# Windere/EAS-SNN

Hardware: AMD Instinct MI355X
Metric: event-frames/sec (T=3) SYOLOX-S Gen1 304x240 (higher is better)
Workload: dtype f32

## Files before the change

### eas_snn_amd/csrc/conv_wgrad_mfma.hip

```cpp
#include <stdio.h>
#include <stdlib.h>

#include "eas_common.h"

namespace {

typedef __bf16 bf16x8 __attribute__((ext_vector_type(8)));
typedef short s16x4 __attribute__((ext_vector_type(4)));
typedef float f32x16 __attribute__((ext_vector_type(16)));
typedef __attribute__((address_space(3))) s16x4 lds_s16x4;

constexpr int TP = 80;
constexpr int KST = TP / 16;
#ifndef EAS_WG_COMMIT_KS
#define EAS_WG_COMMIT_KS (KST - 2)
#endif
constexpr int COMMIT_KS = EAS_WG_COMMIT_KS;
constexpr int ROWB = 64;
constexpr int A_PLANE = TP * ROWB;

__device__ __attribute__((aligned(16))) float eas_wg_zero_page[4] = {0.f, 0.f, 0.f, 0.f};

struct WgGeom {
    int NI, Cin, Cout, Hi, Wi, Ho, Wo;
    int RT, rows_seg, nseg, rows_in, RS, Q;
    int total_rows, ntiles, kslices;
    int ci_blocks;
    int pitchX, pitchY;
    int parts, Wst, lpad, qshift, hv;
    int pn;
    int single;
    int nit;
};

__device__ __forceinline__ void split3(float v, __bf16& hi, __bf16& mid, __bf16& lo) {
    hi = (__bf16)v;
    const float r1 = v - (float)hi;
    mid = (__bf16)r1;
    const float r2 = r1 - (float)mid;
    lo = (__bf16)r2;
}

__device__ __forceinline__ bf16x8 tr_frag(const unsigned char* p0, const unsigned char* p1) {
    const s16x4 a = __builtin_amdgcn_ds_read_tr16_b64_v4i16((lds_s16x4*)p0);
    const s16x4 b = __builtin_amdgcn_ds_read_tr16_b64_v4i16((lds_s16x4*)p1);
    return __builtin_bit_cast(bf16x8, __builtin_shufflevector(a, b, 0, 1, 2, 3, 4, 5, 6, 7));
}

template <int NTERMS>
__device__ __forceinline__ void stage_terms(unsigned char* dst, int term_stride, const float (&v)[8]) {
    if constexpr (NTERMS == 1) {
        bf16x8 t0;
#pragma unroll
        for (int j = 0; j < 8; ++j) t0[j] = (__bf16)v[j];
        *(bf16x8*)dst = t0;
    } else {
        bf16x8 t0, t1, t2;
#pragma unroll
        for (int j = 0; j < 8; ++j) {
            __bf16 a, b, c;
            split3(v[j], a, b, c);
            t0[j] = a;
            t1[j] = b;
            t2[j] = c;
        }
        *(bf16x8*)dst = t0;
        *(bf16x8*)(dst + term_stride) = t1;
        *(bf16x8*)(dst + 2 * term_stride) = t2;
    }
}

template <int S, int XT, int PM, int PN, int VEC, bool XPL, int NITX = 0>
__device__ __forceinline__ void conv_wgrad_body(const float* __restrict__ x, const float* __restrict__ gy, float* __restrict__ slabs,
                                                const WgGeom& g, unsigned char* smem, const int bx, const int by) {
    static_assert(!XPL || XT == 1, "spike planes are one exact bf16 term");
    typedef float vecf __attribute__((ext_vector_type(VEC)));
    typedef unsigned int u32x4 __attribute__((ext_vector_type(4)));
    constexpr int NW = 3 * PM * PN, NT = 64 * NW, NIT = NITX ? NITX : (PM * PN == 4 ? 1 : 2);
    constexpr int A_TERM = PM * A_PLANE, A_BYTES = 3 * A_TERM;
    const int tid = threadIdx.x, lane = tid & 63, wave = tid >> 6;
    const int kh = wave % 3, pair = wave / 3, pm = pair / PN, pn = pair % PN;
    const int cob = by / g.ci_blocks, cib = by - cob * g.ci_blocks;
    const int co0 = cob * 32 * PM, ci0 = cib * 32 * PN;
    const int b_plane = g.Q * ROWB, b_term = PN * b_plane;
    const int buf_bytes = A_BYTES + XT * b_term;
    const int npix = g.RT * g.Wo;

    if (g.parts == 1) {
        const int rows = g.nseg * g.rows_in;
        for (int i = tid; i < rows * 2 * 4 * PN * XT * (g.single ? 1 : 2); i += NT) {
            int rest = i;
            const int piece = rest & 3; rest >>= 2;
            const int side = rest & 1; rest >>= 1;
            const int row = rest % rows; rest /= rows;
            const int pl = rest % (PN * XT), buf = rest / (PN * XT);
            const int col = side ? g.RS - 1 : 0;
            *(uint4*)(smem + (size_t)buf * buf_bytes + A_BYTES + (size_t)pl * b_plane + ((size_t)row * g.RS + col) * ROWB + piece * 16) =
                make_uint4(0, 0, 0, 0);
        }
    }

    if (PN == 1 && g.Cin - ci0 < 32) {
        const int ng = (g.Cin - ci0 + 7) / 8;
        for (int i = tid; i < g.Q * (4 - ng) * XT * (g.single ? 1 : 2); i += NT) {
            int rest = i;
            const int grp = ng + rest % (4 - ng); rest /= (4 - ng);
            const int q = rest % g.Q; rest /= g.Q;
            const int t = rest % XT, buf = rest / XT;
            *(uint4*)(smem + (size_t)buf * buf_bytes + A_BYTES + (size_t)t * b_term + (size_t)q * ROWB + grp * 16) = make_uint4(0, 0, 0, 0);
        }
    }

    const int gq = lane >> 4, li = lane & 15, qrow = li >> 2, pcol = li & 3;
    const int lane_col_bytes = ((gq & 1) * 16 + 4 * pcol) * 2;
    const int kb = (gq >> 1) * 8 + qrow;
    const int a_lane = pm * A_PLANE + kb * ROWB + lane_col_bytes;
    int b_lane[KST][2];
#pragma unroll
    for (int ks = 0; ks < KST; ++ks)
#pragma unroll
        for (int rd = 0; rd < 2; ++rd) {
            const int p = ks * 16 + kb + 4 * rd;
            int q = 0;
            if (p < npix) {
                const int rl = p / g.Wo, c = p - rl * g.Wo;
                const int seg = rl / g.rows_seg, rr = rl - seg * g.rows_seg;
                q = (seg * g.rows_in + rr * S) * g.RS + c * S + g.qshift;
            }
            b_lane[ks][rd] = A_BYTES + pn * b_plane + q * ROWB + lane_col_bytes;
        }

    const int unitsA = TP / VEC, nA = unitsA * 4 * PM;
    const int nbg = PN == 1 ? (g.Cin - ci0 >= 32 ? 4 : (g.Cin - ci0 + 7) / 8) : 4 * PN;
    const int units_row = g.Wst / VEC, units_seg = g.rows_in * units_row, unitsB = g.nseg * units_seg, nB = unitsB * nbg;
    const int part = g.parts > 1 ? bx % g.parts : 0;
    const int ycol0 = part * g.Wo;
    const int xcol0 = g.parts > 1 ? ycol0 * S - g.hv : 0;
    const int nitems = nA + nB;
    const size_t planeY = (size_t)g.Ho * g.pitchY, planeX = (size_t)g.Hi * g.pitchX;
    constexpr bool BUF = XT == 1;
    constexpr unsigned OOB = 0x80000000u;
    int it_kind[NIT], it_seg[NIT], it_row[NIT], it_lofs[NIT];
    unsigned it_off[BUF ? NIT : 1];
    int it_col[BUF ? 1 : NIT], it_ch[BUF ? 1 : NIT];
#pragma unroll
    for (int it = 0; it < NIT; ++it) {
        int id = it * NT + tid;
        id = id < nitems ? id : nitems - 1;
        if (id < nA) {
            const int u = id / (4 * PM), gi = id - u * (4 * PM);
            const int p0 = u * VEC;
            const int rl = p0 / g.Wo, c = p0 - rl * g.Wo;
            it_kind[it] = p0 < npix ? 0 : 2;
            it_seg[it] = rl / g.rows_seg;
            it_row[it] = rl - it_seg[it] * g.rows_seg;
            const int ch = co0 + gi * 8;
            if constexpr (BUF) {
                it_off[it] = (p0 < npix && ch < g.Cout)
                                 ? (unsigned)((((size_t)it_seg[it] * g.Cout + ch) * g.Ho + it_row[it]) * g.pitchY + ycol0 + c) * 4u : OOB;
            } else {
                it_col[it] = c;
                it_ch[it] = gi * 8;
            }
            it_lofs[it] = (gi >> 2) * A_PLANE + p0 * ROWB + (gi & 3) * 16;
        } else {
            const int idb = id - nA;
            const int u = idb / nbg, gi = idb - u * nbg;
            const int seg = u / units_seg, rem = u - seg * units_seg;
            const int rl = rem / units_row, cu = rem - rl * units_row;
            it_kind[it] = 1;
            it_seg[it] = seg;
            it_row[it] = rl;
            const int ch = ci0 + gi * 8, gc = xcol0 + cu * VEC;
            if constexpr (BUF) {
                const bool sok = ch < g.Cin && gc >= 0 && gc < g.pitchX;
                it_off[it] = !sok ? OOB
                             : XPL ? (unsigned)((((size_t)seg * (g.Cin / 8) + (ch >> 3)) * g.Hi + rl) * g.pitchX + gc) * 16u
                                   : (unsigned)((((size_t)seg * g.Cin + ch) * g.Hi + rl) * g.pitchX + gc) * 4u;
            } else {
                it_col[it] = cu * VEC;
                it_ch[it] = gi * 8;
            }
            it_lofs[it] = A_BYTES + (gi >> 2) * b_plane + ((seg * g.rows_in + rl) * g.RS + g.lpad + cu * VEC) * ROWB + (gi & 3) * 16;
        }
    }

    vecf L[NIT][8];
    constexpr bool UNI = NIT == 1;
    u32x4 LP[UNI ? 1 : NIT][(XPL && !UNI) ? VEC : 1];
    const unsigned planeYb = (unsigned)planeY * 4u, planeXb = (unsigned)planeX * 4u;
    auto fetch = [&](int it, int tile) {
        const int rho0 = (g.parts > 1 ? tile / g.parts : tile) * g.RT;
        const int img0 = rho0 / g.Ho, r0 = rho0 - img0 * g.Ho;
        if constexpr (!BUF) {
            const int img = img0 + it_seg[it];
            const float* src;
            size_t plane;
            bool ok;
            if (it_kind[it] == 1) {
                const int ir = r0 * S - 1 + it_row[it];
                const int gc = xcol0 + it_col[it];
                ok = ir >= 0 && ir < g.Hi && img < g.NI && ci0 + it_ch[it] < g.Cin && gc >= 0 && gc < g.pitchX;
                const int ch = ci0 + it_ch[it] < g.Cin ? ci0 + it_ch[it] : g.Cin - 8;
                src = x + (((size_t)(ok ? img : 0) * g.Cin + ch) * g.Hi + (ok ? ir : 0)) * g.pitchX + (ok ? gc : 0);
                plane = planeX;
            } else {
                ok = it_kind[it] == 0 && img < g.NI && co0 + it_ch[it] < g.Cout;
                const int ch = co0 + it_ch[it] < g.Cout ? co0 + it_ch[it] : g.Cout - 8;
                src = gy + (((size_t)(ok ? img : 0) * g.Cout + ch) * g.Ho + (ok ? r0 + it_row[it] : 0)) * g.pitchY + (ok ? ycol0 + it_col[it] : 0);
                plane = planeY;
            }
            const float* sp = ok ? src : eas_wg_zero_page;
            const size_t cs = ok ? plane : 0;
#pragma unroll
            for (int j = 0; j < 8; ++j) L[it][j] = *(const vecf*)(sp + j * cs);
        } else {
        const bool img_ok = img0 + it_seg[it] < g.NI;
        if (it_kind[it] == 1) {
            const int r0s = r0 * S - 1;
            const bool ok = img_ok && (unsigned)(r0s + it_row[it]) < (unsigned)g.Hi;
            const unsigned voff = ok ? it_off[it] : OOB;
            if constexpr (XPL) {
                const char* base = reinterpret_cast<const char*>(x) + (((long)img0 * (g.Cin / 8)) * g.Hi + r0s) * (long)g.pitchX * 16;
                const __amdgpu_buffer_rsrc_t rs = __builtin_amdgcn_make_buffer_rsrc((void*)base, 0, OOB, 0x00020000);
#pragma unroll
                for (int p = 0; p < VEC; ++p) {
                    const u32x4 v = __builtin_amdgcn_raw_buffer_load_b128(rs, voff + 16 * p, 0, 0);
                    if constexpr (!UNI) {
                        LP[it][p] = v;
                    } else if constexpr (VEC == 4) {
                        L[it][p] = __builtin_bit_cast(vecf, v);
                    } else {
                        typedef unsigned int u32x2 __attribute__((ext_vector_type(2)));
                        L[it][2 * p] = __builtin_bit_cast(vecf, (u32x2)__builtin_shufflevector(v, v, 0, 1));
                        L[it][2 * p + 1] = __builtin_bit_cast(vecf, (u32x2)__builtin_shufflevector(v, v, 2, 3));
                    }
                }
            } else {
                const char* base = reinterpret_cast<const char*>(x) + (((long)img0 * g.Cin) * g.Hi + r0s) * (long)g.pitchX * 4;
                const __amdgpu_buffer_rsrc_t rs = __builtin_amdgcn_make_buffer_rsrc((void*)base, 0, OOB, 0x00020000);
#pragma unroll
                for (int j = 0; j < 8; ++j) {
                    if constexpr (VEC == 4) L[it][j] = __builtin_bit_cast(vecf, __builtin_amdgcn_raw_buffer_load_b128(rs, voff, j * planeXb, 0));
                    else L[it][j] = __builtin_bit_cast(vecf, __builtin_amdgcn_raw_buffer_load_b64(rs, voff, j * planeXb, 0));
                }
            }
        } else {
            const unsigned voff = img_ok ? it_off[it] : OOB;
            const char* base = reinterpret_cast<const char*>(gy) + (((long)img0 * g.Cout) * g.Ho + r0) * (long)g.pitchY * 4;
            const __amdgpu_buffer_rsrc_t rs = __builtin_amdgcn_make_buffer_rsrc((void*)base, 0, OOB, 0x00020000);
#pragma unroll
            for (int j = 0; j < 8; ++j) {
                if constexpr (VEC == 4) L[it][j] = __builtin_bit_cast(vecf, __builtin_amdgcn_raw_buffer_load_b128(rs, voff, j * planeYb, 0));
                else L[it][j] = __builtin_bit_cast(vecf, __builtin_amdgcn_raw_buffer_load_b64(rs, voff, j * planeYb, 0));
            }
        }
        }
    };
    auto commit = [&](unsigned char* buf, int it) {
        if (XPL && it_kind[it] == 1) {
#pragma unroll
            for (int p = 0; p < VEC; ++p) {
                if constexpr (!UNI) {
                    *(u32x4*)(buf + it_lofs[it] + p * ROWB) = LP[it][p];
                } else if constexpr (VEC == 4) {
                    *(vecf*)(buf + it_lofs[it] + p * ROWB) = L[it][p];
                } else {
                    *(vecf*)(buf + it_lofs[it] + p * ROWB) = L[it][2 * p];
                    *(vecf*)(buf + it_lofs[it] + p * ROWB + 8) = L[it][2 * p + 1];
                }
            }
            return;
        }
#pragma unroll
        for (int p = 0; p < VEC; ++p) {
            float v[8];
#pragma unroll
            for (int j = 0; j < 8; ++j) v[j] = L[it][j][p];
            unsigned char* dst = buf + it_lofs[it] + p * ROWB;
            if (it_kind[it] == 1) stage_terms<XT>(dst, b_term, v);
            else stage_terms<3>(dst, A_TERM, v);
        }
    };

    f32x16 acc[3];
#pragma unroll
    for (int t = 0; t < 3; ++t)
#pragma unroll
        for (int e = 0; e < 16; ++e) acc[t][e] = 0.0f;

    int tile = bx;
    if (tile < g.ntiles) {
#pragma unroll
        for (int it = 0; it < NIT; ++it)
            if (it * NT < nitems) fetch(it, tile);
#pragma unroll
        for (int it = 0; it < NIT; ++it)
            if (it * NT < nitems) commit(smem, it);
    }
    __syncthreads();

    const bool single = g.single != 0;
    int par = 0;
    for (; tile < g.ntiles; tile += g.kslices, par ^= (single ? 0 : 1)) {
        const unsigned char* cur = smem + par * buf_bytes;
        unsigned char* nxt = smem + (single ? 0 : (par ^ 1)) * buf_bytes;
        const bool more = tile + g.kslices < g.ntiles;
#pragma unroll
        for (int ks = 0; ks < KST; ++ks) {
            if (ks == 0 && more) {
#pragma unroll
                for (int it = 0; it < NIT; ++it)
                    if (it * NT < nitems) fetch(it, tile + g.kslices);
            }
            __builtin_amdgcn_sched_barrier(0);
            bf16x8 a[3];
#pragma unroll
            for (int t = 0; t < 3; ++t) {
                const unsigned char* pa = cur + a_lane + t * A_TERM + ks * 16 * ROWB;
                a[t] = tr_frag(pa, pa + 4 * ROWB);
            }
#pragma unroll
            for (int kw = 0; kw < 3; ++kw) {
                const int toff = (kh * g.RS + kw) * ROWB;
                bf16x8 b[XT];
#pragma unroll
                for (int t = 0; t < XT; ++t) b[t] = tr_frag(cur + b_lane[ks][0] + toff + t * b_term, cur + b_lane[ks][1] + toff + t * b_term);
                if constexpr (XT == 1) {
                    acc[kw] = __builtin_amdgcn_mfma_f32_32x32x16_bf16(a[2], b[0], acc[kw], 0, 0, 0);
                    acc[kw] = __builtin_amdgcn_mfma_f32_32x32x16_bf16(a[1], b[0], acc[kw], 0, 0, 0);
                    acc[kw] = __builtin_amdgcn_mfma_f32_32x32x16_bf16(a[0], b[0], acc[kw], 0, 0, 0);
                } else {
                    acc[kw] = __builtin_amdgcn_mfma_f32_32x32x16_bf16(a[2], b[0], acc[kw], 0, 0, 0);
                    acc[kw] = __builtin_amdgcn_mfma_f32_32x32x16_bf16(a[0], b[2], acc[kw], 0, 0, 0);
                    acc[kw] = __builtin_amdgcn_mfma_f32_32x32x16_bf16(a[1], b[1], acc[kw], 0, 0, 0);
                    acc[kw] = __builtin_amdgcn_mfma_f32_32x32x16_bf16(a[1], b[0], acc[kw], 0, 0, 0);
                    acc[kw] = __builtin_amdgcn_mfma_f32_32x32x16_bf16(a[0], b[1], acc[kw], 0, 0, 0);
                    acc[kw] = __builtin_amdgcn_mfma_f32_32x32x16_bf16(a[0], b[0], acc[kw], 0, 0, 0);
                }
            }
            if (ks == COMMIT_KS && more && !single) {
#pragma unroll
                for (int it = 0; it < NIT; ++it)
                    if (it * NT < nitems) commit(nxt, it);
            }
        }
        if (single && more) {
            __syncthreads();
#pragma unroll
            for (int it = 0; it < NIT; ++it)
                if (it * NT < nitems) commit(nxt, it);
        }
        __syncthreads();
    }

    const int ci = ci0 + pn * 32 + (lane & 31);
    float* slab = slabs + (size_t)bx * g.Cout * g.Cin * 9;
    if (ci < g.Cin) {
        const int cob = co0 + pm * 32 + 4 * (lane >> 5);
        float* d0 = slab + ((size_t)cob * g.Cin + ci) * 9 + kh * 3;
        const size_t rs = (size_t)g.Cin * 9;
        const bool full = co0 + pm * 32 + 32 <= g.Cout;
#pragma unroll
        for (int e = 0; e < 16; ++e) {
            if (full || cob + (e & 3) + 8 * (e >> 2) < g.Cout) {
                float* d = d0 + ((e & 3) + 8 * (e >> 2)) * rs;
                d[0] = acc[0][e];
                d[1] = acc[1][e];
                d[2] = acc[2][e];
            }
        }
    }
}

template <int S, int XT, int PM, int PN, int VEC, bool XPL = false, int NITX = 0>
__global__ __launch_bounds__(192 * PM * PN) void conv_wgrad_mfma_kernel(const float* __restrict__ x, const float* __restrict__ gy,
                                                                        float* __restrict__ slabs, WgGeom g) {
    extern __shared__ __align__(16) unsigned char smem[];
    conv_wgrad_body<S, XT, PM, PN, VEC, XPL, NITX>(x, gy, slabs, g, smem, (int)blockIdx.x, (int)blockIdx.y);
}

constexpr int kMaxWgGroup = 8;
struct WgGroupArgs {
    WgGeom g[kMaxWgGroup];
    const float* x[kMaxWgGroup];
    const float* gy[kMaxWgGroup];
    float* slabs[kMaxWgGroup];
    int first[kMaxWgGroup + 1];
    int vec2[kMaxWgGroup];
    int n;
};

template <int XT, int PM, int PN>
__global__ __launch_bounds__(192 * PM * PN) void conv_wgrad_group_kernel(const WgGroupArgs a) {
    extern __shared__ __align__(16) unsigned char smem[];
    int p = 0;
    for (int i = 1; i < a.n; ++i)
        if ((int)blockIdx.x >= a.first[i]) p = i;
    p = __builtin_amdgcn_readfirstlane(p);
    const int lb = (int)blockIdx.x - a.first[p];
    const int ks = a.g[p].kslices, by = lb / ks, bx = lb - by * ks;
    if (a.vec2[p]) conv_wgrad_body<1, XT, PM, PN, 2, false>(a.x[p], a.gy[p], a.slabs[p], a.g[p], smem, bx, by);
    else conv_wgrad_body<1, XT, PM, PN, 4, false>(a.x[p], a.gy[p], a.slabs[p], a.g[p], smem, bx, by);
}

__device__ __forceinline__ void wgrad_reduce_block(const float* __restrict__ slabs, float* __restrict__ gw, int n, int kslices, int block) {
    __shared__ double part[4][64][4];
    const int o = threadIdx.x & 63, kl = threadIdx.x >> 6;
    const bool v4 = (n & 3) == 0 && (((uintptr_t)slabs | (uintptr_t)gw) & 15) == 0;
    const int per = v4 ? 4 : 1;
    const int i = (block * 64 + o) * per;
    double s[4] = {0.0, 0.0, 0.0, 0.0};
    if (i < n) {
        int k = kl;
        if (v4) {
            for (; k + 28 < kslices; k += 32) {
                float4 v[8];
#pragma unroll
                for (int u = 0; u < 8; ++u) v[u] = *reinterpret_cast<const float4*>(slabs + (size_t)(k + 4 * u) * n + i);
#pragma unroll
                for (int u = 0; u < 8; ++u) {
                    s[0] += (double)v[u].x; s[1] += (double)v[u].y; s[2] += (double)v[u].z; s[3] += (double)v[u].w;
                }
            }
            for (; k < kslices; k += 4) {
                const float4 v = *reinterpret_cast<const float4*>(slabs + (size_t)k * n + i);
                s[0] += (double)v.x; s[1] += (double)v.y; s[2] += (double)v.z; s[3] += (double)v.w;
            }
        } else {
            for (; k + 12 < kslices; k += 16) {
                const float a = slabs[(size_t)k * n + i], b = slabs[(size_t)(k + 4) * n + i], c = slabs[(size_t)(k + 8) * n + i],
                            d = slabs[(size_t)(k + 12) * n + i];
                s[0] += (double)a;
                s[0] += (double)b;
                s[0] += (double)c;
                s[0] += (double)d;
            }
            for (; k < kslices; k += 4) s[0] += (double)slabs[(size_t)k * n + i];
        }
    }
#pragma unroll
    for (int j = 0; j < 4; ++j) part[kl][o][j] = s[j];
    __syncthreads();
    if (kl == 0 && i < n) {
        if (v4) {
            float4 r;
            r.x = (float)(((part[0][o][0] + part[1][o][0]) + part[2][o][0]) + part[3][o][0]);
            r.y = (float)(((part[0][o][1] + part[1][o][1]) + part[2][o][1]) + part[3][o][1]);
            r.z = (float)(((part[0][o][2] + part[1][o][2]) + part[2][o][2]) + part[3][o][2]);
            r.w = (float)(((part[0][o][3] + part[1][o][3]) + part[2][o][3]) + part[3][o][3]);
            *reinterpret_cast<float4*>(gw + i) = r;
        } else {
            gw[i] = (float)(((part[0][o][0] + part[1][o][0]) + part[2][o][0]) + part[3][o][0]);
        }
    }
}

static inline int wgrad_reduce_blocks(const float* slabs, const float* gw, int n) {
    const bool v4 = (n & 3) == 0 && (((uintptr_t)slabs | (uintptr_t)gw) & 15) == 0;
    return (n + (v4 ? 256 : 64) - 1) / (v4 ? 256 : 64);
}

__global__ __launch_bounds__(256) void conv_wgrad_reduce_kernel(const float* __restrict__ slabs, float* __restrict__ gw, int n, int kslices) {
    wgrad_reduce_block(slabs, gw, n, kslices, (int)blockIdx.x);
}

constexpr int kReduceJobsPerLaunch = 96;
struct ReduceJobs {
    const float* slabs[kReduceJobsPerLaunch];
    float* gw[kReduceJobsPerLaunch];
    int n[kReduceJobsPerLaunch];
    int kslices[kReduceJobsPerLaunch];
    int first_block[kReduceJobsPerLaunch + 1];
    int njobs;
};

__global__ __launch_bounds__(256) void conv_wgrad_reduce_many_kernel(const ReduceJobs jobs) {
    int lo = 0, hi = jobs.njobs;
    while (hi - lo > 1) {
        const int mid = (lo + hi) >> 1;
        if (jobs.first_block[mid] <= (int)blockIdx.x) lo = mid; else hi = mid;
    }
    wgrad_reduce_block(jobs.slabs[lo], jobs.gw[lo], jobs.n[lo], jobs.kslices[lo], (int)blockIdx.x - jobs.first_block[lo]);
}

constexpr size_t kWgLdsMax = 160 * 1024;

int pick_rows(int Ho, int Wo, int cap) {
    int best = 0;
    for (int rt = 1; rt * Wo <= cap; ++rt)
        if (Ho % rt == 0 || rt % Ho == 0) best = rt;
    return best;
}

struct WgInst { int s, xt, pm, pn, vec, nit; bool planes; };

constexpr int wg_nit(int pm, int pn, int nitx) { return nitx ? nitx : (pm * pn == 4 ? 1 : 2); }

WgInst wg_inst(const WgGeom& g, int stride, int x_terms, bool planes, int pn, int nitx) {
    WgInst in;
    in.s = stride; in.xt = x_terms; in.planes = planes;
    in.pm = g.Cout >= 64 ? 2 : 1;
    in.pn = pn;
    in.vec = (g.parts > 1 || (g.Wi % 4 == 0 && g.Wo % 4 == 0)) ? 4 : 2;
    in.nit = wg_nit(in.pm, pn, nitx);
    return in;
}

struct WgFit {
    size_t lds;
    int nitems, capacity;
    bool ok() const { return lds <= kWgLdsMax && nitems <= capacity; }
};
WgFit wg_fit(const WgGeom& g, const WgInst& in, bool single) {
    WgFit f;
    f.lds = (size_t)(single ? 1 : 2) * (3 * in.pm * A_PLANE + (size_t)in.xt * in.pn * g.Q * ROWB);
    const int nbg = in.pn == 1 && g.Cin < 32 ? (g.Cin + 7) / 8 : 4 * in.pn;
    f.nitems = (TP / in.vec) * 4 * in.pm + g.nseg * g.rows_in * (g.Wst / in.vec) * nbg;
    f.capacity = in.nit * 192 * in.pm * in.pn;
    return f;
}

bool wg_geom_cap(WgGeom& g, int NI, int Cin, int Cout, int Hi, int Wi, int stride, int cap, int parts) {
    g.NI = NI; g.Cin = Cin; g.Cout = Cout; g.Hi = Hi; g.Wi = Wi;
    g.Ho = (Hi + 2 - 3) / stride + 1;
    const int WoF = (Wi + 2 - 3) / stride + 1;
    g.parts = parts;
    g.pitchX = Wi; g.pitchY = WoF;
    if (parts == 1) {
        g.Wo = WoF; g.Wst = Wi; g.lpad = 1; g.qshift = 0; g.hv = 0;
        g.RS = Wi + 2;
    } else {
        if (WoF % parts != 0 || Wi % 4 != 0 || ((WoF / parts) * stride) % 4 != 0 || (WoF / parts) % 4 != 0 || WoF * stride != Wi) return false;
        g.Wo = WoF / parts; g.hv = 4; g.Wst = g.Wo * stride + 2 * g.hv; g.lpad = 0; g.qshift = g.hv - 1;
        g.RS = g.Wst;
    }
    g.RT = pick_rows(g.Ho, g.Wo, cap);
    if (g.RT == 0) return false;
    g.rows_seg = g.RT < g.Ho ? g.RT : g.Ho;
    g.nseg = g.RT / g.rows_seg;
    g.rows_in = (g.rows_seg - 1) * stride + 3;
    g.Q = g.nseg * g.rows_in * g.RS;
    g.total_rows = NI * g.Ho;
    g.ntiles = ((g.total_rows + g.RT - 1) / g.RT) * parts;
    return true;
}

bool wg_geom(WgGeom& g, WgInst& in, int NI, int Cin, int Cout, int Hi, int Wi, int stride, int x_terms, bool planes) {
    static const int force_parts = eas_dev_env("EAS_WG_PARTS") ? atoi(eas_dev_env("EAS_WG_PARTS")) : 0;
    static const int pn2_s2 = eas_dev_env("EAS_WG_PN2_S2") ? atoi(eas_dev_env("EAS_WG_PN2_S2")) : 1;
    for (int parts = force_parts > 0 ? force_parts : 1; parts <= 8; parts *= 2) {
        for (int cap = TP; cap >= 8; cap /= 2)
          for (int pn = (Cin >= 64 && x_terms == 1 && (stride == 1 || (pn2_s2 && cap == TP))) ? 2 : 1; pn >= 1; --pn) {
            if (!wg_geom_cap(g, NI, Cin, Cout, Hi, Wi, stride, cap, parts)) continue;
            in = wg_inst(g, stride, x_terms, planes, pn, 0);
            bool ok = wg_fit(g, in, false).ok();
            if (!ok && stride == 2 && x_terms == 1 && in.pm == 2 && pn == 1 && cap == TP) {
                in = wg_inst(g, stride, x_terms, planes, pn, 3);
                ok = wg_fit(g, in, false).ok();
            }
            if (ok) {
                g.pn = in.pn;
                g.nit = in.nit;
                return true;
            }
        }
        if (force_parts > 0) break;
    }
    return false;
}

int wg_support(WgGeom& g, WgInst& in, int NI, int Cin, int Cout, int Hi, int Wi, int stride, int x_terms) {
    if (NI <= 0 || Cin <= 0 || Cout <= 0 || Hi <= 0 || Wi <= 0) return EAS_ERR_INVALID_ARG;
    if (x_terms < 1 || x_terms > 3 || (stride != 1 && stride != 2)) return EAS_ERR_UNSUPPORTED;
    if (Cin % 8 != 0 || Cout % 8 != 0 || Wi % 2 != 0) return EAS_ERR_UNSUPPORTED;
    const bool planes = x_terms == 2;
    if (!wg_geom(g, in, NI, Cin, Cout, Hi, Wi, stride, planes ? 1 : x_terms, planes)) return EAS_ERR_UNSUPPORTED;
    if (g.Wo % 2 != 0 || (g.Ho * g.pitchY) % 4 != 0) return EAS_ERR_UNSUPPORTED;
    if (in.xt == 1) {
        const size_t img_y = (size_t)g.Cout * g.Ho * g.pitchY * 4, img_x = (size_t)g.Cin * g.Hi * g.pitchX * (planes ? 2 : 4);
        const size_t span = (size_t)(g.nseg + 1) * (img_y > img_x ? img_y : img_x) + (size_t)8 * g.Hi * g.pitchX * 4;
        if (span >= ((size_t)1 << 31)) return EAS_ERR_UNSUPPORTED;
    }
    return EAS_OK;
}

template <auto KERN>
bool wg_raise_lds() {
    static bool raised = false;
    if (!raised) raised = hipFuncSetAttribute((const void*)KERN, hipFuncAttributeMaxDynamicSharedMemorySize, (int)kWgLdsMax) == hipSuccess;
    return raised;
}

template <auto KERN>
int wg_resident(int threads, size_t lds) {
    static size_t seen[16];
    static int val[16], n = 0;
    for (int i = 0; i < n; ++i)
        if (seen[i] == lds) return val[i];
    (void)wg_raise_lds<KERN>();
    int nb = 0;
    if (hipOccupancyMaxActiveBlocksPerMultiprocessor(&nb, (const void*)KERN, threads, lds) != hipSuccess || nb < 1) nb = 1;
    if (n < 16) { seen[n] = lds; val[n] = nb; ++n; }
    return nb;
}

struct WgCall {
    const float* x;
    const float* gy;
    float* slabs;
    WgGeom g;
    WgInst in;
    hipStream_t st;
};

template <int S, int XT, int PM, int PN, int VEC, bool XPL, int NITX>
int wg_instance(const WgCall* c, size_t lds) {
    constexpr auto kern = conv_wgrad_mfma_kernel<S, XT, PM, PN, VEC, XPL, NITX>;
    constexpr int NT = 192 * PM * PN;
    if (!c) return wg_resident<kern>(NT, lds);
    const WgInst& in = c->in;
    if (in.s != S || in.xt != XT || in.pm != PM || in.pn != PN || in.vec != VEC || in.planes != XPL || in.nit != wg_nit(PM, PN, NITX))
        return EAS_ERR_LAUNCH;
    if (!wg_raise_lds<kern>()) return EAS_ERR_LAUNCH;
    dim3 grid(c->g.kslices, ((c->g.Cout + 32 * PM - 1) / (32 * PM)) * c->g.ci_blocks);
    EAS_LAUNCH(kern, grid, dim3(NT), lds, c->st, c->x, c->gy, c->slabs, c->g);
    return EAS_OK;
}

struct WgRow {
    WgInst in;
    int (*fn)(const WgCall*, size_t);
};
template <int S, int XT, int PM, int PN, int VEC, bool XPL = false, int NITX = 0>
constexpr WgRow wg_row() {
    return {{S, XT, PM, PN, VEC, wg_nit(PM, PN, NITX), XPL}, wg_instance<S, XT, PM, PN, VEC, XPL, NITX>};
}
const WgRow kWgLadder[] = {
    wg_row<1, 1, 1, 1, 2>(), wg_row<1, 1, 1, 1, 4>(), wg_row<1, 1, 1, 2, 2>(), wg_row<1, 1, 1, 2, 4>(),
    wg_row<1, 1, 2, 1, 2>(), wg_row<1, 1, 2, 1, 4>(), wg_row<1, 1, 2, 2, 2>(), wg_row<1, 1, 2, 2, 4>(),
    wg_row<1, 1, 1, 1, 2, true>(), wg_row<1, 1, 1, 1, 4, true>(), wg_row<1, 1, 1, 2, 2, true>(), wg_row<1, 1, 1, 2, 4, true>(),
    wg_row<1, 1, 2, 1, 2, true>(), wg_row<1, 1, 2, 1, 4, true>(), wg_row<1, 1, 2, 2, 2, true>(), wg_row<1, 1, 2, 2, 4, true>(),
    wg_row<1, 3, 1, 1, 2>(), wg_row<1, 3, 1, 1, 4>(), wg_row<1, 3, 2, 1, 2>(), wg_row<1, 3, 2, 1, 4>(),
    wg_row<2, 1, 1, 1, 2>(), wg_row<2, 1, 1, 1, 4>(), wg_row<2, 1, 1, 2, 2>(), wg_row<2, 1, 1, 2, 4>(),
    wg_row<2, 1, 2, 1, 2>(), wg_row<2, 1, 2, 1, 4>(), wg_row<2, 1, 2, 2, 2>(), wg_row<2, 1, 2, 2, 4>(),
    wg_row<2, 1, 1, 1, 2, true>(), wg_row<2, 1, 1, 1, 4, true>(), wg_row<2, 1, 1, 2, 2, true>(), wg_row<2, 1, 1, 2, 4, true>(),
    wg_row<2, 1, 2, 1, 2, true>(), wg_row<2, 1, 2, 1, 4, true>(), wg_row<2, 1, 2, 2, 2, true>(), wg_row<2, 1, 2, 2, 4, true>(),
    wg_row<2, 3, 1, 1, 2>(), wg_row<2, 3, 1, 1, 4>(), wg_row<2, 3, 2, 1, 2>(), wg_row<2, 3, 2, 1, 4>(),
    wg_row<2, 1, 2, 1, 2, false, 3>(), wg_row<2, 1, 2, 1, 2, true, 3>(),
};

int wg_select(const WgInst& in, const WgCall* c, size_t lds) {
    for (const WgRow& r : kWgLadder)
        if (r.in.s == in.s && r.in.xt == in.xt && r.in.pm == in.pm && r.in.pn == in.pn && r.in.vec == in.vec && r.in.nit == in.nit &&
            r.in.planes == in.planes)
            return r.fn(c, lds);
    return EAS_ERR_UNSUPPORTED;
}

long wg_slots(int resident) {
    static const int slot_pct = eas_dev_env("EAS_WG_SLOT_PCT") ? atoi(eas_dev_env("EAS_WG_SLOT_PCT")) : 100;
    return 256L * resident * slot_pct / 100;
}

int wg_slices(const WgGeom& g, const WgInst& in, int resident) {
    const int yz = ((g.Cout + 32 * in.pm - 1) / (32 * in.pm)) * ((g.Cin + 32 * in.pn - 1) / (32 * in.pn));
    const long slots = wg_slots(resident);
    const int step = g.parts > 1 ? g.parts : 1;
    int best = step;
    static const double pen = eas_dev_env("EAS_WG_SHARE_PEN") ? atof(eas_dev_env("EAS_WG_SHARE_PEN")) : 0.0;
    double best_cost = -1.0;
    for (int ks = step; ks <= g.ntiles && (long)ks * yz <= 4L * slots; ks += step) {
        const long blocks = (long)ks * yz;
        const long rounds = (blocks + slots - 1) / slots;
        long share = (blocks + 255) / 256;
        if (share > resident) share = resident;
        const double cost = (double)rounds * (double)((g.ntiles + ks - 1) / ks) * (1.0 + pen * (double)(share - 1));
        if (best_cost < 0 || cost < best_cost - 1e-9) { best_cost = cost; best = ks; }
    }
    return best;
}

struct WgPlan { int kslices, single; };

WgPlan wg_plan(const WgGeom& g, const WgInst& in) {
    const size_t lds = wg_fit(g, in, false).lds;
    int res = wg_select(in, nullptr, lds);
    if (res < 1) return {0, 0};
    static const int single_env = eas_dev_env("EAS_WG_SINGLE") ? atoi(eas_dev_env("EAS_WG_SINGLE")) : -1;
    int single = 0;
    static const int single_cap = eas_dev_env("EAS_WG_SINGLE_CAP") ? atoi(eas_dev_env("EAS_WG_SINGLE_CAP")) : 2;
    if (single_env != 0 && res == 1 && in.nit != 3 && (in.pm * in.pn == 1 || single_env == 1)) {
        const int res1 = wg_select(in, nullptr, wg_fit(g, in, true).lds);
        if (res1 >= 2) {
            single = 1;
            res = res1 > single_cap ? single_cap : res1;
        }
    }
    return {wg_slices(g, in, res), single};
}


template <int PM>
int wg_group_instance(const WgGroupArgs* a, int blocks, size_t lds, hipStream_t st) {
    constexpr auto kern = conv_wgrad_group_kernel<3, PM, 1>;
    if (!a) return wg_resident<kern>(192 * PM, lds);
    if (!wg_raise_lds<kern>()) return EAS_ERR_LAUNCH;
    EAS_LAUNCH(kern, dim3(blocks), dim3(192 * PM), lds, st, *a);
    return EAS_OK;
}
int wg_group_select(int pm, const WgGroupArgs* a, int blocks, size_t lds, hipStream_t st) {
    return pm == 2 ? wg_group_instance<2>(a, blocks, lds, st) : wg_group_instance<1>(a, blocks, lds, st);
}

int group_tau(const int* yz, const int* nt, int n, long slots) {
    int max_nt = 0;
    for (int p = 0; p < n; ++p) max_nt = nt[p] > max_nt ? nt[p] : max_nt;
    int best = max_nt;
    long best_cost = -1;
    for (int tau = max_nt; tau >= 1; --tau) {
        long blocks = 0;
        for (int p = 0; p < n; ++p) blocks += (long)((nt[p] + tau - 1) / tau) * yz[p];
        if (blocks > 4 * slots && best_cost >= 0) break;
        const long cost = ((blocks + slots - 1) / slots) * tau;
        if (best_cost < 0 || cost < best_cost) { best_cost = cost; best = tau; }
    }
    return best;
}

int wgrad_group3(const EasWgradProblem* pr, int n, int x_terms, hipStream_t st, int* slabs_out, bool query) {
    if (n > kMaxWgGroup || x_terms != 3) return EAS_ERR_UNSUPPORTED;
    WgGroupArgs a{};
    int yz[kMaxWgGroup], nt[kMaxWgGroup];
    size_t lds = 0;
    int pm = 0;
    for (int p = 0; p < n; ++p) {
        const EasWgradProblem& q = pr[p];
        if (!query && (!q.x || !q.grad_y || !q.workspace)) return EAS_ERR_INVALID_ARG;
        WgGeom& g = a.g[p];
        WgInst in;
        const int rc = wg_support(g, in, q.NI, q.Cin, q.Cout, q.Hi, q.Wi, 1, x_terms);
        if (rc != EAS_OK) return rc;
        if (p == 0) pm = in.pm;
        if (g.parts != 1 || in.pn != 1 || in.pm != pm) return EAS_ERR_UNSUPPORTED;
        a.vec2[p] = in.vec == 2;
        const size_t l = wg_fit(g, in, false).lds;
        lds = l > lds ? l : lds;
        g.ci_blocks = (g.Cin + 31) / 32;
        yz[p] = ((g.Cout + 32 * pm - 1) / (32 * pm)) * g.ci_blocks;
        nt[p] = g.ntiles;
        a.x[p] = (const float*)q.x; a.gy[p] = q.grad_y; a.slabs[p] = q.workspace;
    }
    const int res = wg_group_select(pm, nullptr, 0, lds, st);
    const int tau = group_tau(yz, nt, n, wg_slots(res));
    int blocks = 0;
    for (int p = 0; p < n; ++p) {
        a.g[p].kslices = (nt[p] + tau - 1) / tau;
        a.g[p].single = 0;
        if (slabs_out) slabs_out[p] = a.g[p].kslices;
        a.first[p] = blocks;
        blocks += a.g[p].kslices * yz[p];
    }
    a.first[n] = blocks;
    a.n = n;
    if (query) return EAS_OK;
    return wg_group_select(pm, &a, blocks, lds, st);
}

}

int eas_conv1x1_wgrad_group(const EasWgradProblem* pr, int n, int x_terms, hipStream_t st, int* slabs_out, bool query);
int eas_conv1x1_wgrad_slices(int NI, int Cin, int Cout, int HW, int x_terms, int planes);
int eas_conv1x1_wgrad_dispatch(const void* x, const float* gy, float* slabs, int NI, int Cin, int Cout, int HW, int x_terms, hipStream_t st,
                               int planes);

extern "C" {

int64_t eas_conv_wgrad_workspace_floats(int NI, int Cin, int Cout, int Hi, int Wi, int ksize, int stride, int x_terms) {
    if (ksize == 1) {
        const bool planes = x_terms == 2;
        return stride == 1 ? (int64_t)eas_conv1x1_wgrad_slices(NI, Cin, Cout, Hi * Wi, planes ? 1 : x_terms, planes ? 1 : 0) * Cout * Cin : 0;
    }
    if (ksize != 3) return 0;
    WgGeom g{};
    WgInst in;
    if (wg_support(g, in, NI, Cin, Cout, Hi, Wi, stride, x_terms) != EAS_OK) return 0;
    return (int64_t)wg_plan(g, in).kslices * Cout * Cin * 9;
}

int eas_conv_wgrad_parts(int NI, int Cin, int Cout, int Hi, int Wi, int stride, int x_terms) {
    WgGeom g{};
    WgInst in;
    return wg_support(g, in, NI, Cin, Cout, Hi, Wi, stride, x_terms) == EAS_OK ? g.parts : 0;
}

static int wgrad_partial(const float* x, const float* grad_y, float* workspace, int NI, int Cin, int Cout, int Hi, int Wi, int ksize,
                         int stride, int x_terms, eas_stream_t stream) {
    if (!x || !grad_y || !workspace || NI <= 0 || Cin <= 0 || Cout <= 0 || Hi <= 0 || Wi <= 0) return EAS_ERR_INVALID_ARG;
    const bool planes = x_terms == 2;
    if (planes) x_terms = 1;
    if ((x_terms != 1 && x_terms != 3) || (planes && (Cin % 8 != 0 || ((uintptr_t)x & 15)))) return EAS_ERR_UNSUPPORTED;
    if (ksize == 1) {
        if (stride != 1) return EAS_ERR_UNSUPPORTED;
        EAS_CLEAR_ERR();
        const int slices = eas_conv1x1_wgrad_slices(NI, Cin, Cout, Hi * Wi, x_terms, planes ? 1 : 0);
        if (slices <= 0) return EAS_ERR_UNSUPPORTED;
        const int rc1 = eas_conv1x1_wgrad_dispatch(x, grad_y, workspace, NI, Cin, Cout, Hi * Wi, x_terms, eas_s(stream), planes ? 1 : 0);
        if (rc1 != EAS_OK) return rc1;
        EAS_CHECK_LAUNCH();
        return slices;
    }
    if (ksize != 3) return EAS_ERR_UNSUPPORTED;
    EAS_CLEAR_ERR();
    WgCall c{x, grad_y, workspace, {}, {}, eas_s(stream)};
    const int rc = wg_support(c.g, c.in, NI, Cin, Cout, Hi, Wi, stride, planes ? 2 : x_terms);
    if (rc != EAS_OK) return rc;
    const WgPlan p = wg_plan(c.g, c.in);
    if (p.kslices < 1) return EAS_ERR_UNSUPPORTED;
    c.g.kslices = p.kslices;
    c.g.single = p.single;
    c.g.ci_blocks = (Cin + 32 * c.in.pn - 1) / (32 * c.in.pn);
    const WgFit f = wg_fit(c.g, c.in, p.single != 0);
    if (!f.ok()) {
        if (eas_dev_env("EAS_CONV_DBG"))
            fprintf(stderr, "wgrad launch: lds %zu nitems %d of %d PM %d PN %d VEC %d RT %d Q %d\n", f.lds, f.nitems, f.capacity, c.in.pm, c.in.pn, c.in.vec, c.g.RT, c.g.Q);
        return EAS_ERR_UNSUPPORTED;
    }
    const int rcl = wg_select(c.in, &c, f.lds);
    if (rcl != EAS_OK) return rcl;
    EAS_CHECK_LAUNCH();
    return p.kslices;
}

int eas_conv_wgrad(const float* x, const float* grad_y, float* grad_w, float* workspace, int NI, int Cin, int Cout, int Hi, int Wi, int ksize,
                   int stride, int x_terms, eas_stream_t stream) {
    if (!grad_w) return EAS_ERR_INVALID_ARG;
    const int slabs = wgrad_partial(x, grad_y, workspace, NI, Cin, Cout, Hi, Wi, ksize, stride, x_terms, stream);
    if (slabs < 0) return slabs;
    const int n = Cout * Cin * ksize * ksize;
    EAS_LAUNCH(conv_wgrad_reduce_kernel, dim3(wgrad_reduce_blocks(workspace, grad_w, n)), dim3(256), 0, eas_s(stream), workspace, grad_w, n, slabs);
    EAS_CHECK_LAUNCH();
    return EAS_OK;
}

int eas_conv_wgrad_partial(const float* x, const float* grad_y, float* workspace, int NI, int Cin, int Cout, int Hi, int Wi, int ksize,
                           int stride, int x_terms, eas_stream_t stream) {
    if (x_terms == 2) return EAS_ERR_INVALID_ARG;
    return wgrad_partial(x, grad_y, workspace, NI, Cin, Cout, Hi, Wi, ksize, stride, x_terms, stream);
}

int eas_conv_wgrad_planes_partial(const void* x_planes, const float* grad_y, float* workspace, int NI, int Cin, int Cout, int Hi, int Wi, int ksize,
                                  int stride, eas_stream_t stream) {
    return wgrad_partial(reinterpret_cast<const float*>(x_planes), grad_y, workspace, NI, Cin, Cout, Hi, Wi, ksize, stride, 2, stream);
}

static int wgrad_group_impl(const EasWgradProblem* pr, int n, int ksize, int x_terms, eas_stream_t stream, int* slabs_out, bool query) {
    if (!pr || n < 1) return EAS_ERR_INVALID_ARG;
    if (ksize != 1 && ksize != 3) return EAS_ERR_UNSUPPORTED;
    EAS_CLEAR_ERR();
    const int rc = ksize == 1 ? eas_conv1x1_wgrad_group(pr, n, x_terms, eas_s(stream), slabs_out, query)
                              : wgrad_group3(pr, n, x_terms, eas_s(stream), slabs_out, query);
    if (rc != EAS_OK || query) return rc;
    EAS_CHECK_LAUNCH();
    return EAS_OK;
}

int eas_conv_wgrad_group_plan(const EasWgradProblem* problems, int n, int ksize, int x_terms, int* slabs_out) {
    return wgrad_group_impl(problems, n, ksize, x_terms, nullptr, slabs_out, true);
}

int eas_conv_wgrad_group_partial(const EasWgradProblem* problems, int n, int ksize, int x_terms, eas_stream_t stream) {
    return wgrad_group_impl(problems, n, ksize, x_terms, stream, nullptr, false);
}

int eas_conv_wgrad_reduce_many(const EasWgradReduceJob* jobs, int njobs, eas_stream_t stream) {
    if (!jobs || njobs < 1) return EAS_ERR_INVALID_ARG;
    EAS_CLEAR_ERR();
    for (int j0 = 0; j0 < njobs; j0 += kReduceJobsPerLaunch) {
        ReduceJobs a;
        a.njobs = njobs - j0 < kReduceJobsPerLaunch ? njobs - j0 : kReduceJobsPerLaunch;
        int blocks = 0;
        for (int j = 0; j < a.njobs; ++j) {
            const EasWgradReduceJob& q = jobs[j0 + j];
            if (!q.slabs || !q.grad_w || q.n < 1 || q.slabs_count < 1) return EAS_ERR_INVALID_ARG;
            a.slabs[j] = q.slabs; a.gw[j] = q.grad_w; a.n[j] = q.n; a.kslices[j] = q.slabs_count;
            a.first_block[j] = blocks;
            blocks += wgrad_reduce_blocks(q.slabs, q.grad_w, q.n);
        }
        a.first_block[a.njobs] = blocks;
        EAS_LAUNCH(conv_wgrad_reduce_many_kernel, dim3(blocks), dim3(256), 0, eas_s(stream), a);
        EAS_CHECK_LAUNCH();
    }
    return EAS_OK;
}

}
```

Before: 3470.

## Add PM=4 wgrad tiles with single-buffered x planes for stride-2 spike layers

Adds a PM=4 instantiation of the 3x3 weight-gradient MFMA kernel that covers 128 output channels per block. In this mode the grad_y (A) tiles stay double-buffered while the x-plane tile is single-buffered and committed after a barrier, which keeps LDS usage within limits. A planner step switches stride-2 spike-plane layers with Cout>64 to this variant when the launch would need more blocks than there are resident slots. The intent is fewer blocks and more reuse of each loaded x tile across output channels. The cost is an extra __syncthreads per tile and less overlap of x loads with compute.

```diff
diff --git a/eas_snn_amd/csrc/conv_wgrad_mfma.hip b/eas_snn_amd/csrc/conv_wgrad_mfma.hip
--- a/eas_snn_amd/csrc/conv_wgrad_mfma.hip
+++ b/eas_snn_amd/csrc/conv_wgrad_mfma.hip
@@ -85,10 +85,12 @@
     const int b_plane = g.Q * ROWB, b_term = PN * b_plane;
     const int buf_bytes = A_BYTES + XT * b_term;
     const int npix = g.RT * g.Wo;
+    constexpr bool XONE = PM == 4;
+    const int xbufs = (XONE || g.single) ? 1 : 2;
 
     if (g.parts == 1) {
         const int rows = g.nseg * g.rows_in;
-        for (int i = tid; i < rows * 2 * 4 * PN * XT * (g.single ? 1 : 2); i += NT) {
+        for (int i = tid; i < rows * 2 * 4 * PN * XT * xbufs; i += NT) {
             int rest = i;
             const int piece = rest & 3; rest >>= 2;
             const int side = rest & 1; rest >>= 1;
@@ -102,7 +104,7 @@
 
     if (PN == 1 && g.Cin - ci0 < 32) {
         const int ng = (g.Cin - ci0 + 7) / 8;
-        for (int i = tid; i < g.Q * (4 - ng) * XT * (g.single ? 1 : 2); i += NT) {
+        for (int i = tid; i < g.Q * (4 - ng) * XT * xbufs; i += NT) {
             int rest = i;
             const int grp = ng + rest % (4 - ng); rest /= (4 - ng);
             const int q = rest % g.Q; rest /= g.Q;
@@ -304,6 +306,7 @@
     int par = 0;
     for (; tile < g.ntiles; tile += g.kslices, par ^= (single ? 0 : 1)) {
         const unsigned char* cur = smem + par * buf_bytes;
+        const unsigned char* curx = XONE ? smem : cur;
         unsigned char* nxt = smem + (single ? 0 : (par ^ 1)) * buf_bytes;
         const bool more = tile + g.kslices < g.ntiles;
 #pragma unroll
@@ -325,7 +328,7 @@
                 const int toff = (kh * g.RS + kw) * ROWB;
                 bf16x8 b[XT];
 #pragma unroll
-                for (int t = 0; t < XT; ++t) b[t] = tr_frag(cur + b_lane[ks][0] + toff + t * b_term, cur + b_lane[ks][1] + toff + t * b_term);
+                for (int t = 0; t < XT; ++t) b[t] = tr_frag(curx + b_lane[ks][0] + toff + t * b_term, curx + b_lane[ks][1] + toff + t * b_term);
                 if constexpr (XT == 1) {
                     acc[kw] = __builtin_amdgcn_mfma_f32_32x32x16_bf16(a[2], b[0], acc[kw], 0, 0, 0);
                     acc[kw] = __builtin_amdgcn_mfma_f32_32x32x16_bf16(a[1], b[0], acc[kw], 0, 0, 0);
@@ -342,8 +345,14 @@
             if (ks == COMMIT_KS && more && !single) {
 #pragma unroll
                 for (int it = 0; it < NIT; ++it)
-                    if (it * NT < nitems) commit(nxt, it);
-            }
+                    if (it * NT < nitems && !(XONE && it_kind[it] == 1)) commit(nxt, it);
+            }
+        }
+        if (XONE && more) {
+            __syncthreads();
+#pragma unroll
+            for (int it = 0; it < NIT; ++it)
+                if (it * NT < nitems && it_kind[it] == 1) commit(smem, it);
         }
         if (single && more) {
             __syncthreads();
@@ -514,7 +523,8 @@
 };
 WgFit wg_fit(const WgGeom& g, const WgInst& in, bool single) {
     WgFit f;
-    f.lds = (size_t)(single ? 1 : 2) * (3 * in.pm * A_PLANE + (size_t)in.xt * in.pn * g.Q * ROWB);
+    const size_t ay = (size_t)3 * in.pm * A_PLANE, bx = (size_t)in.xt * in.pn * g.Q * ROWB;
+    f.lds = in.pm == 4 ? 2 * ay + bx : (size_t)(single ? 1 : 2) * (ay + bx);
     const int nbg = in.pn == 1 && g.Cin < 32 ? (g.Cin + 7) / 8 : 4 * in.pn;
     f.nitems = (TP / in.vec) * 4 * in.pm + g.nseg * g.rows_in * (g.Wst / in.vec) * nbg;
     f.capacity = in.nit * 192 * in.pm * in.pn;
@@ -648,6 +658,7 @@
     wg_row<2, 1, 2, 1, 2, true>(), wg_row<2, 1, 2, 1, 4, true>(), wg_row<2, 1, 2, 2, 2, true>(), wg_row<2, 1, 2, 2, 4, true>(),
     wg_row<2, 3, 1, 1, 2>(), wg_row<2, 3, 1, 1, 4>(), wg_row<2, 3, 2, 1, 2>(), wg_row<2, 3, 2, 1, 4>(),
     wg_row<2, 1, 2, 1, 2, false, 3>(), wg_row<2, 1, 2, 1, 2, true, 3>(),
+    wg_row<2, 1, 4, 1, 4, true>(), wg_row<2, 1, 4, 1, 2, true, 2>(),
 };
 
 int wg_select(const WgInst& in, const WgCall* c, size_t lds) {
@@ -681,12 +692,12 @@
     return best;
 }
 
-struct WgPlan { int kslices, single; };
+struct WgPlan { int kslices, single, resident; };
 
 WgPlan wg_plan(const WgGeom& g, const WgInst& in) {
     const size_t lds = wg_fit(g, in, false).lds;
     int res = wg_select(in, nullptr, lds);
-    if (res < 1) return {0, 0};
+    if (res < 1) return {0, 0, 0};
     static const int single_env = eas_dev_env("EAS_WG_SINGLE") ? atoi(eas_dev_env("EAS_WG_SINGLE")) : -1;
     int single = 0;
     static const int single_cap = eas_dev_env("EAS_WG_SINGLE_CAP") ? atoi(eas_dev_env("EAS_WG_SINGLE_CAP")) : 2;
@@ -697,7 +708,28 @@
             res = res1 > single_cap ? single_cap : res1;
         }
     }
-    return {wg_slices(g, in, res), single};
+    return {wg_slices(g, in, res), single, res};
+}
+
+bool wg_coblocks(WgGeom& g, WgInst& in, WgPlan& p) {
+    const char* sw = getenv("EAS_WG_COBLOCKS");
+    if (sw && sw[0] == '0') return false;
+    if (in.s != 2 || in.pm != 2 || in.pn != 1 || g.Cout <= 64 || !in.planes) return false;
+    const long blocks = (long)p.kslices * ((g.Cout + 63) / 64) * ((g.Cin + 31) / 32);
+    if (!(sw && sw[0] == '1') && blocks <= wg_slots(p.resident)) return false;
+    WgInst w = in;
+    w.pm = 4;
+    for (w.nit = 1; w.nit <= 2; ++w.nit) {
+        const WgFit f = wg_fit(g, w, false);
+        if (f.lds > kWgLdsMax) return false;
+        if (f.ok() && wg_select(w, nullptr, f.lds) >= 1) {
+            in = w;
+            g.nit = w.nit;
+            p.single = 0;
+            return true;
+        }
+    }
+    return false;
 }
 
 
@@ -815,8 +847,9 @@
     WgCall c{x, grad_y, workspace, {}, {}, eas_s(stream)};
     const int rc = wg_support(c.g, c.in, NI, Cin, Cout, Hi, Wi, stride, planes ? 2 : x_terms);
     if (rc != EAS_OK) return rc;
-    const WgPlan p = wg_plan(c.g, c.in);
+    WgPlan p = wg_plan(c.g, c.in);
     if (p.kslices < 1) return EAS_ERR_UNSUPPORTED;
+    (void)wg_coblocks(c.g, c.in, p);
     c.g.kslices = p.kslices;
     c.g.single = p.single;
     c.g.ci_blocks = (Cin + 32 * c.in.pn - 1) / (32 * c.in.pn);
```

Result: no change. 3469 (-0.0%).
